# 5l1v3r1/gr-dvbt2ll

Hardware: NVIDIA B200
Metric: t2_baseband_msps (higher is better)
Workload: dtype u8/f32

## Files before the change

gr-dvbt2ll_b200/csrc/t2_capi.cu:

```cuda
#include "../../include/dvbt2ll_cuda.h"

#include <cuda_runtime.h>

#include <algorithm>
#include <cmath>
#include <cstdio>
#include <cstdlib>
#include <cstring>
#include <memory>
#include <mutex>
#include <string>
#include <vector>

#include "t2_kernels.cuh"
#include "t2_plan.h"

namespace {

thread_local std::string g_err;

int fail(int code, const std::string &msg) { g_err = msg; return code; }

#define CK(call)                                                                                  \
  do {                                                                                            \
// ... 549 lines not shown
    t2k::GatherArgs a;
    a.in = (const float2 *)d_in; a.in_stride = plan.stream_items;
    a.out = (float2 *)d_out; a.out_stride = plan.mapped_items;
    a.code = d_code.as<int32_t>(); a.n = plan.mapped_items; a.pool = d_pool.as<float2>();
    a.l1post_base = plan.pool.l1post_base; a.l1post_cells = plan.pool.l1post_cells; a.l1post_variants = plan.pool.l1post_variants;
    a.frames = frames; a.frame_idx0 = t2_frame_num;
    t2k::launch_gather(a, s);
    CK(cudaGetLastError());
    t2_frame_num = (t2_frame_num + frames) % plan.prm.t2frames;
    if (consumed) *consumed = frames * plan.stream_items;
    return frames * plan.mapped_items;
  }
  long long plan_get(const char *name, void *out, long long cap) const
  {
    std::string n(name);
    if (n == "frame.code") return copy_vec(plan.code, out, cap);
    if (n == "frame.pool") return copy_vec(plan.pool.cells, out, cap);
    if (n == "frame.cell_perm") return copy_vec(plan.cell_perm, out, cap);
    if (n == "frame.fec_shift") return copy_vec(plan.fec_shift, out, cap);
    if (n == "frame.ci_dst") return copy_vec(plan.ci_dst, out, cap);
    if (n == "frame.ti_src") return copy_vec(plan.ti_src, out, cap);
    if (n == "frame.dims") return dims_get(plan.dims, out, cap);
    if (n == "frame.info") {
      const int v[12] = { plan.cell_size, plan.stream_items, plan.mapped_items, plan.eta_mod, plan.n_post, plan.n_punc,
                          plan.dummy_cells, plan.pool.l1post_base, plan.pool.l1post_cells, plan.pool.l1post_variants,
                          plan.pool_dummy, plan.pool_zero };
      return copy_out(v, sizeof(v), out, cap);
    }
    return -1;
  }
};

struct OfdmDevice {
  DevBuf d_code, d_pool, d_p1, d_sinc, d_tw, d_tw_split, d_scratch, d_sym_flags;
  int log2_m, split;
  long long pool_stride;
  long long scratch_slot_elems;
  int init(const std::vector<int32_t> &code, const t2::CellPool &pool, const t2::OfdmPlan &op, bool c16 = false)
  {
    {
      const int nv = pool.l1post_variants > 0 ? pool.l1post_variants : 1;
      pool_stride = (long long)pool.cells.size();
      std::vector<t2::cfloat> rep((size_t)nv * pool.cells.size());
      for (int v = 0; v < nv; v++) {
        std::copy(pool.cells.begin(), pool.cells.end(), rep.begin() + (size_t)v * pool.cells.size());
        for (int i = 0; i < pool.l1post_cells; i++)
          rep[(size_t)v * pool.cells.size() + pool.l1post_base + i] = pool.cells[pool.l1post_base + (size_t)v * pool.l1post_cells + i];
      }
      CK(upload(d_pool, rep));
    }
    CK(upload(d_p1, op.p1));
    const int N = op.dims.fft_n;
    split = N > 16384 ? 2 : 1;
    {
      const char *e = std::getenv("DVBT2LL_OFDM_SPLIT16K");
      if (c16 && N == 16384 && e && e[0] == '1') split = 2;
    }
    scratch_slot_elems = 0;
    const int M = N / split;
    log2_m = 0;
    while ((1 << log2_m) < M) log2_m++;
    const int L = op.dims.num_symbols, cps = op.dims.c_ps;
    std::vector<int> pos(M);
    for (int m = 0; m < M; m++) pos[m] = t2k::ofdm_table_index(t2k::ofdm_position_of_bin(m, log2_m), log2_m);
    std::vector<int32_t> code_pos((size_t)L * N, -1);
    std::vector<int32_t> sym_flags(L, 0);
    for (int l = 0; l < L; l++)
      for (int p = 0; p < split; p++)
        for (int m = 0; m < M; m++) {
          const int c = (split * m + p + N / 2) & (N - 1);
          const int k = c - op.left_nulls;
          int32_t v = (k >= 0 && k < cps) ? code[(size_t)l * cps + k] : -1;
          if (c16) {
            if (v >= 0) {
              if (v >= 65536) return fail(DVBT2LL_ERR_INVALID, "chain: staging slot out of range");
              v = 2 * v;
            }
            else if (~v < 8) v = (~v + 1) << 17;
            else { v = (int32_t)(0x80000000u | (uint32_t)(~v)); sym_flags[l] = 1; }
          }
          code_pos[((size_t)l * split + p) * M + pos[m]] = v;
        }
    CK(upload(d_code, code_pos));
    CK(upload(d_sym_flags, sym_flags));
    if (!op.inv_sinc.empty()) {
      std::vector<float> sinc_pos((size_t)N);
      for (int p = 0; p < split; p++)
        for (int m = 0; m < M; m++) sinc_pos[(size_t)p * M + pos[m]] = op.inv_sinc[(split * m + p + N / 2) & (N - 1)];
      CK(upload(d_sinc, sinc_pos));
    }
    CK(upload(d_tw, make_twiddles(M, M)));
    if (split == 2) {
      CK(upload(d_tw_split, make_twiddles(N, M)));
      int dev = 0, sms = 148;
      cudaGetDevice(&dev);
      cudaDeviceGetAttribute(&sms, cudaDevAttrMultiProcessorCount, dev);
      scratch_slot_elems = (long long)(4 * sms + 8) * M;
      CK(d_scratch.ensure((size_t)2 * scratch_slot_elems * sizeof(float2)));
    }
    return 0;
  }
  void fill(t2k::OfdmArgs &a, const t2::OfdmPlan &op, const t2::CellPool &pool) const
  {
    a.code_pos = d_code.as<int32_t>(); a.pool = d_pool.as<float2>(); a.pool_stride = pool_stride;
    a.l1post_base = pool.l1post_base; a.l1post_cells = pool.l1post_cells; a.l1post_variants = pool.l1post_variants;
    a.p1 = d_p1.as<float2>(); a.sinc_pos = op.inv_sinc.empty() ? 0 : d_sinc.as<float>();
    a.tw = d_tw.as<float2>(); a.tw_split = split == 2 ? d_tw_split.as<float2>() : 0;
    a.fft_n = op.dims.fft_n; a.log2_m = log2_m; a.split = split;
    a.c_ps = op.dims.c_ps; a.left_nulls = op.left_nulls; a.gi = op.dims.gi; a.num_symbols = op.dims.num_symbols;
    a.norm = op.normalization;
    a.cells16 = 0; a.run_desc = 0; a.run_ptr = 0; a.run_cnt = 0; a.desc_cap = 0; a.stage_bytes = 0; a.stage_cap = 0; a.lut = 0; a.lut_n = 0; a.lut_single = 0;
    a.sym_flags = d_sym_flags.as<int32_t>();
    a.out_fmt = 0; a.sink_gain = 1.0f; a.scratch = d_scratch.as<float2>();
    a.cells_len = 0; a.out_len = 0; a.pool_len = pool_stride;
  }
};

struct OfdmHandle : dvbt2ll_handle {
  t2::OfdmPlan plan;
  OfdmDevice dev;
  OfdmHandle() : dvbt2ll_handle(OFDM) {}
  int output_multiple() const { return plan.samples_per_frame; }
  int in_item() const { return 8; }
  int out_item() const { return 8; }
  int forecast(int noutput) const { return plan.dims.active_items * (noutput / plan.samples_per_frame); }
  int dev_init() { return dev.init(plan.code, plan.pool, plan); }
  int work_device(const void *d_in, int ninput, void *d_out, int noutput, int *consumed, cudaStream_t s)
  {
    const int frames = noutput / plan.samples_per_frame;
    if (consumed) *consumed = 0;
    if (frames < 1) return 0;
    if ((long long)ninput < (long long)frames * plan.dims.active_items)
      return fail(DVBT2LL_ERR_SHORT, "pilotgenp1insert_cc: not enough input items");
    t2k::OfdmArgs a;
    dev.fill(a, plan, plan.pool);
    a.cells = (const float2 *)d_in; a.cells_stride = plan.dims.active_items;
    a.out = d_out; a.out_stride = plan.samples_per_frame;
    a.cells_len = (long long)frames * plan.dims.active_items; a.out_len = (long long)frames * plan.samples_per_frame;
    a.frames = frames; a.frame_idx0 = 0; a.frames_per_channel = frames;
    t2k::launch_ofdm(a, s);
    CK(cudaGetLastError());
    if (consumed) *consumed = frames * plan.dims.active_items;
    return frames * plan.samples_per_frame;
  }
  long long plan_get(const char *name, void *out, long long cap) const
  {
// ... 86 lines not shown
    int r;
    if ((r = bb.dev_init())) return r;
    if ((r = ldpc.dev_init())) return r;
    if ((r = map.dev_init())) return r;
    if ((r = odev.init(tables.code, tables.pool, oplan, true))) return r;
    CK(upload(d_ci_inv, fplan.cell_perm_inv));
    {
      const int nc = (int)fplan.cell_perm_inv.size();
      ci4_stride = (nc + 8 + 3) & ~3;
      std::vector<uint16_t> c4((size_t)4 * ci4_stride, 0);
      for (int k = 0; k < 4; k++)
        for (int j = 0; j + k < nc; j++) {
          const int c = fplan.cell_perm_inv[j + k];
          c4[(size_t)k * ci4_stride + j] = (uint16_t)(c + 2 * (c >> 6));
        }
      CK(upload(d_ci_inv4, c4));
    }
    CK(upload(d_fec_shift, fplan.fec_shift));
    CK(upload(d_run_desc, tables.run_desc));
    CK(upload(d_run_ptr, tables.run_ptr));
    CK(upload(d_run_cnt, tables.run_cnt));
    CK(upload(d_stage_bytes, tables.stage_bytes));
    stage_cap = (tables.max_slots + 7) & ~7;
    if ((size_t)(1 << odev.log2_m) * 8 * 17 / 16 + (size_t)stage_cap * 2 + 2048 + 96 + (size_t)(tables.max_runs + 2) * 8 > 227 * 1024)
      return fail(DVBT2LL_ERR_INVALID, "chain: the cells of one OFDM symbol do not fit the shared-memory staging area");
    const size_t nfec = (size_t)max_frames * F();
    CK(d_bch.ensure(nfec * align16(bb.plan.fec.nbch / 8) + 64));
    CK(d_cells.ensure((size_t)max_frames * cells16_stride() * sizeof(uint16_t) + 64));
    CK(cudaMemset(d_cells.p, 0, (size_t)max_frames * cells16_stride() * sizeof(uint16_t) + 64));
    for (int s = 0; s < TIMING_SLOTS; s++) for (int i = 0; i < 5; i++) CK(cudaEventCreate(&ev[s][i]));
    return 0;
  }
  int run(const void *d_ts, long long ts_pitch, int n_channels, int n_frames, long long first_frame, void *d_out, cudaStream_t s,
          int buf_frame = 0, int scratch_slot = 0, int hist_valid = -1)
  {
    const int frames = n_channels * n_frames;
    if (frames < 1) return 0;
    if (buf_frame + frames > max_frames) return fail(DVBT2LL_ERR_INVALID, "chain: batch larger than max_frames given at create");
    const int nfec = frames * F();
    const int bp = align16(bb.plan.fec.nbch / 8), fp = align16(bb.plan.fec.nldpc / 8);
    cudaEvent_t *tev = ev[n_timed % TIMING_SLOTS];
    if (timing) cudaEventRecord(tev[0], s);
    uint8_t *bch_buf = d_bch.as<uint8_t>() + (size_t)buf_frame * F() * bp;
    if (!fuse_fec || taps) CK(d_fec.ensure((size_t)max_frames * F() * fp + 64));
    uint8_t *fec_buf = d_fec.as<uint8_t>() ? d_fec.as<uint8_t>() + (size_t)buf_frame * F() * fp : 0;
    uint16_t *cell_buf = d_cells.as<uint16_t>() + (size_t)buf_frame * cells16_stride();
    for (int pl = 0; pl < P(); pl++) {
      const int fpl = Fp(pl);
      const long long j0 = first_frame * fpl;
      const int fb0 = bb.plan.inband ? (int)(j0 % fpl) : 0;
      const int count0 = (int)(stream_pos(first_frame, pl) % 188);
      t2k::BbArgs ba;
      bb.fill_args(ba, (const uint8_t *)d_ts + (long long)pl * ts_pitch, ts_pitch * P(), n_channels, n_frames * fpl, count0, fb0,
                   hist_valid >= 0 ? hist_valid : (first_frame > 0 ? 1 : 0), bch_buf, bp);
      ba.fecblocks = fpl;
      ba.ts_len = ts_bytes(first_frame, n_frames, pl);
      ba.out_len = (long long)frames * F() * bp;
      if (P() > 1) { ba.out_group = fpl; ba.out_group_stride = F(); ba.out_group_off = fplan.plp_first_block[pl]; }
      t2k::launch_bb_bch(ba, s);
    }
    if (timing) cudaEventRecord(tev[1], s);
    t2k::LdpcArgs la;
    ldpc.fill_args(la, bch_buf, bp, fec_buf, fp, nfec);
    t2k::MapArgs ma;
    map.fill_args(ma, fec_buf, fp, 0, nfec);
    ma.out16 = cell_buf; ma.out16_frame_stride = cells16_stride();
    ma.ci_inv = d_ci_inv.as<uint16_t>(); ma.fec_shift = d_fec_shift.as<int32_t>(); ma.fecblocks = F();
    ma.ci_inv4 = d_ci_inv4.as<uint16_t>(); ma.ci_inv4_stride = ci4_stride;
    ma.out_len = (long long)frames * cells16_stride();
    if (fuse_fec) {
      if (timing) cudaEventRecord(tev[2], s);
      t2k::launch_fec(la, ma, taps ? fec_buf : 0, fp, s);
    }
    else {
      t2k::launch_ldpc(la, s);
      if (timing) cudaEventRecord(tev[2], s);
      t2k::launch_map(ma, s);
    }
    if (timing) cudaEventRecord(tev[3], s);
    t2k::OfdmArgs oa;
    odev.fill(oa, oplan, tables.pool);
    oa.cells = 0; oa.cells_stride = cells16_stride();
    oa.cells16 = cell_buf; oa.run_desc = d_run_desc.as<int2>(); oa.run_ptr = d_run_ptr.as<int32_t>();
    oa.run_cnt = d_run_cnt.as<int32_t>(); oa.desc_cap = (tables.max_runs + 2) & ~1;
    oa.stage_bytes = d_stage_bytes.as<int32_t>(); oa.stage_cap = stage_cap; oa.lut_single = map.plan.im_from_re;
    oa.lut = map.d_lut.as<float2>(); oa.lut_n = 1 << map.plan.mod;
    oa.out = d_out; oa.out_stride = oplan.samples_per_frame;
    oa.cells_len = (long long)frames * cells16_stride(); oa.out_len = (long long)frames * oplan.samples_per_frame;
    oa.out_fmt = sink_fmt; oa.sink_gain = sink_gain; oa.norm = oplan.normalization * sink_gain;
    if (oa.scratch && scratch_slot) oa.scratch += odev.scratch_slot_elems;
    oa.frames = frames; oa.frames_per_channel = n_frames;
    oa.frame_idx0 = (int)(first_frame % (tables.pool.l1post_variants > 0 ? tables.pool.l1post_variants : 1));
    t2k::launch_ofdm(oa, s);
    if (timing) { cudaEventRecord(tev[4], s); n_timed++; }
    CK(cudaGetLastError());
    if (buf_frame == 0) last_frames = frames;
    return frames;
  }
  int work_device(const void *d_in, int ninput, void *d_out, int noutput, int *consumed, cudaStream_t s)
  {
    const int frames = noutput / oplan.samples_per_frame;
    if (consumed) *consumed = 0;
    if (frames < 1) return 0;
    const long long need = ts_bytes(next_frame, frames);
    if ((long long)ninput < need) return fail(DVBT2LL_ERR_SHORT, "chain: not enough input items");
    int r = run(d_in, 0, 1, frames, next_frame, d_out, s);
    if (r < 0) return r;
    next_frame += frames;
    if (consumed) *consumed = (int)need;
    return frames * oplan.samples_per_frame;
  }
  long long plan_get(const char *name, void *out, long long cap) const
  {
    std::string n(name);
    if (n == "chain.code") return copy_vec(tables.code, out, cap);
    if (n == "chain.pool") return copy_vec(tables.pool.cells, out, cap);
    if (n == "chain.run_desc") return copy_vec(tables.run_desc, out, cap);
    if (n == "chain.run_ptr") return copy_vec(tables.run_ptr, out, cap);
    if (n == "chain.run_cnt") return copy_vec(tables.run_cnt, out, cap);
    if (n == "chain.stage_bytes") return copy_vec(tables.stage_bytes, out, cap);
    if (n == "ofdm.sym_data_start") return copy_vec(oplan.sym_data_start, out, cap);
    if (n == "frame.framed") return copy_vec(fplan.framed, out, cap);
    if (n == "frame.pool") return copy_vec(fplan.pool.cells, out, cap);
// ... 156 lines not shown
  LinkRec::Slot *mine = 0;
  if (h->link_out) {
    LinkRec &L = *h->link_out;
    mine = &L.slot[L.next];
    if ((r = write_back(L, *mine)) < 0) return r;
    for (int k = 0; k < LinkRec::NSLOT; k++) {
      LinkRec::Slot &S = L.slot[k];
      if (&S != mine && S.valid && (const uint8_t *)out < S.host + S.bytes && (const uint8_t *)out + out_bytes > S.host) {
        if ((r = write_back(L, S)) < 0) return r;
        S.valid = false;
      }
    }
    if (mine->taken_valid) CK(cudaStreamWaitEvent(h->stream, mine->taken_ev, 0));
    mine->valid = false;
    for (int k = 0; k < LinkRec::NSLOT; k++)
      if (!L.slot[k].valid) CK(L.slot[k].buf.ensure(out_bytes + 256));
    lk_out.unlock();
  }
  if (lk_in.owns_lock() && !resident) lk_in.unlock();
  DevBuf &d_out = mine ? mine->buf : h->stage_out;
  if (!resident) CK(d_in.ensure(prefix + in_bytes + 256));
  CK(d_out.ensure(out_bytes + 256));
  uint8_t *din = resident ? const_cast<uint8_t *>(resident) : d_in.as<uint8_t>() + prefix;
  cudaStream_t s = h->stream;
  if (!resident) h->pin(in, in_bytes);
  h->pin(out, out_bytes);
  if (b) {
    CK(cudaMemcpyAsync(din - 187, b->history, 187, cudaMemcpyHostToDevice, s));
    b->hist_on_device = 1;
  }
  if (!resident) CK(h->copy_host(din, in, in_bytes, cudaMemcpyHostToDevice, s));
  int used = 0;
  if (ch) {
    r = ch->run(din, 0, 1, frames, ch->next_frame, d_out.p, s, 0, 0, 1);
    if (r >= 0) { r = nout; used = (int)need; ch->next_frame += frames; }
  }
  else r = h->work_device(din, (int)need, d_out.p, nout, &used, s);
  if (r < 0) return r;
  if (resident) {
    if (!taken->taken_ev) CK(cudaEventCreateWithFlags(&taken->taken_ev, cudaEventDisableTiming));
    CK(cudaEventRecord(taken->taken_ev, s));
    taken->taken_valid = true;
    lk_in.unlock();
  }
  const bool lazy_out = h->link_out && h->link_out->lazy;
  if (!lazy_out) CK(h->copy_host(out, d_out.p, out_bytes, cudaMemcpyDeviceToHost, s));
  CK(cudaStreamSynchronize(s));
  if (b) {
    h->warnings = *b->h_err;
    b->note_consumed((const uint8_t *)in, used);
  }
  if (mine) {
    lk_out.lock();
    LinkRec &L = *h->link_out;
    mine->host = (const uint8_t *)out; mine->bytes = out_bytes; mine->valid = true;
    mine->pending = lazy_out; mine->taken_to = 0;
    L.next = (L.next + 1) % LinkRec::NSLOT;
  }
  if (consumed) *consumed = used;
  return r;
}

long long dvbt2ll_ts_sync(const unsigned char *ts, size_t n)
{
  if (!ts) return -1;
  for (size_t off = 0; off < 188 && off < n; off++) {
    int ok = 0;
// ... 236 lines not shown
{
  ChainHandle *c = as_chain(h);
  if (!c) return fail(DVBT2LL_ERR_INVALID, "not a chain handle");
  int r = c->enter();
  if (r) return r;
  if (n_channels < 0 || n_frames < 0) return fail(DVBT2LL_ERR_INVALID, "chain: negative batch size");
  if (n_channels == 0 || n_frames == 0) return 0;
  const int P = c->P();
  const long long per_ch = c->ts_bytes_max(first_frame, n_frames);
  const long long hist = (first_frame > 0 && c->bb.plan.mode == t2::INPUTMODE_NORMAL) ? 187 : 0;
  if (n_channels * P == 1 && ts_pitch < per_ch + hist) ts_pitch = per_ch + hist;
  if (ts_pitch < per_ch + hist)
    return fail(DVBT2LL_ERR_INVALID, "chain: ts_pitch smaller than the TS bytes (+ 187 history bytes) of one channel");
  const long long dpitch = (per_ch + hist + 255) & ~255LL;
  const size_t ssz = c->sink_fmt ? 4 : 8;
  const size_t out_bytes = (size_t)n_channels * n_frames * c->oplan.samples_per_frame * ssz;
  CK(c->d_ts_stage.ensure((size_t)n_channels * P * dpitch + 512));
  CK(c->d_out_stage.ensure(out_bytes));
  uint8_t *base = c->d_ts_stage.as<uint8_t>() + 256;
  uint8_t *dout = c->d_out_stage.as<uint8_t>();
  const size_t ch_out = (size_t)n_frames * c->oplan.samples_per_frame;
  if (!c->stream2) CK(cudaStreamCreateWithFlags(&c->stream2, cudaStreamNonBlocking));
  int groups = n_channels >= 8 ? 8 : n_channels;
  while (groups > 1 && 2 * ((n_channels + groups - 1) / groups) * n_frames > c->max_frames) groups--;
  const int per = (n_channels + groups - 1) / groups;
  if (2 * per * n_frames > c->max_frames) groups = 1;
  int gi = 0;
  for (int c0 = 0; c0 < n_channels; c0 += (groups == 1 ? n_channels : per), gi++) {
    const int nc = groups == 1 ? n_channels : (c0 + per <= n_channels ? per : n_channels - c0);
    cudaStream_t s = (gi & 1) ? c->stream2 : c->stream;
    CK(cudaMemcpy2DAsync(base + (size_t)c0 * P * dpitch - hist, (size_t)dpitch, (const uint8_t *)ts + (size_t)c0 * P * ts_pitch - hist,
                         (size_t)ts_pitch, (size_t)(per_ch + hist), (size_t)nc * P, cudaMemcpyHostToDevice, s));
    r = c->run(base + (size_t)c0 * P * dpitch, dpitch, nc, n_frames, first_frame, dout + (size_t)c0 * ch_out * ssz, s,
               groups == 1 ? 0 : (gi & 1) * per * n_frames, gi & 1);
    if (r < 0) return r;
    CK(cudaMemcpyAsync((uint8_t *)out + (size_t)c0 * ch_out * ssz, dout + (size_t)c0 * ch_out * ssz, (size_t)nc * ch_out * ssz,
                       cudaMemcpyDeviceToHost, s));
  }
  CK(cudaStreamSynchronize(c->stream));
  CK(cudaStreamSynchronize(c->stream2));
  return n_channels * n_frames;
}

long long dvbt2ll_chain_tap(dvbt2ll_handle *h, const char *stage, void *out, long long cap)
{
  ChainHandle *c = as_chain(h);
  if (!c || !stage) return fail(DVBT2LL_ERR_INVALID, "not a chain handle");
  if (!c->dev_ready || c->last_frames < 1) return fail(DVBT2LL_ERR_INVALID, "chain: nothing has run yet");
  const size_t nfec = (size_t)c->last_frames * c->F();
  const void *src; size_t bytes;
  std::string n(stage);
  if (n == "bch") { src = c->d_bch.p; bytes = nfec * align16(c->bb.plan.fec.nbch / 8); }
  else if (n == "fec") {
    if (c->fuse_fec && !c->taps) return fail(DVBT2LL_ERR_INVALID, "chain: the LDPC codewords stay on chip; call dvbt2ll_chain_enable_taps before the run");
    src = c->d_fec.p; bytes = nfec * align16(c->bb.plan.fec.nldpc / 8);
  }
  else if (n == "cells") { src = c->d_cells.p; bytes = (size_t)c->last_frames * c->cells16_stride() * sizeof(uint16_t); }
  else return fail(DVBT2LL_ERR_INVALID, "chain: unknown tap");
  CK(cudaStreamSynchronize(c->stream));
  CK(cudaDeviceSynchronize());
  if (out && cap > 0) CK(cudaMemcpy(out, src, (size_t)cap < bytes ? (size_t)cap : bytes, cudaMemcpyDeviceToHost));
  return (long long)bytes;
}

int dvbt2ll_chain_set_sink(dvbt2ll_handle *h, int format, float gain)
{
  ChainHandle *c = as_chain(h);
// ... 42 lines not shown
```

gr-dvbt2ll_b200/csrc/t2_kernels.cu:

```cuda
#include "t2_kernels.cuh"

#include <atomic>

#ifdef DVBT2LL_DEBUG_BOUNDS
#include <cstdio>
#define BND(ok)                                                                                                   \
  do {                                                                                                            \
    if (!(ok)) {                                                                                                  \
      printf("DVBT2LL bounds violation: %s (t2_kernels.cu:%d, block %d thread %d)\n", #ok, __LINE__, (int)blockIdx.x, (int)threadIdx.x); \
      __trap();                                                                                                   \
    }                                                                                                             \
  } while (0)
#else
#define BND(ok) do { } while (0)
#endif

namespace t2k {

static std::atomic<long long> g_launches(0);
long long kernel_launch_count() { return g_launches.load(); }
static inline void count_launch() { g_launches.fetch_add(1); }
void count_extra_launch() { count_launch(); }

constexpr int MAX_DEVICES = 64;
// ... 1633 lines not shown
          const unsigned sc = *reinterpret_cast<const uint16_t *>(stage + off);
          const unsigned esh = 2 + lut_rep_shift, emask = 255u << esh, lane_off = (threadIdx.x & ((1u << lut_rep_shift) - 1u)) << 2;
          float2 val = make_float2(*reinterpret_cast<const float *>(reinterpret_cast<const uint8_t *>(lut_re) + (((sc << esh) & emask) | lane_off)),
                                   *reinterpret_cast<const float *>(reinterpret_cast<const uint8_t *>(lut_im) + ((((sc >> 8) << esh) & emask) | lane_off)));
          if (cc >= 0x20000) val = *reinterpret_cast<const float2 *>(spool_m8 + ((unsigned)cc >> 14));
#endif
          if (POOL && cc < 0) val = __ldg(pool + (cc & 0x7FFFFFFF));
          v[b][r] = val;
        }
        else {
          const float2 *base = cc >= 0 ? cells : pool;
          v[b][r] = __ldg(base + (cc >= 0 ? cc : ~cc));
        }
      }
    if (g0 + G::STEP < G::GROUPS) fill_load_codes<LOG2M, T>(code, g0 + G::STEP, c);
#pragma unroll
    for (int b = 0; b < GPB; b++) {
      const int g = g0 + b * T;
      if (SINC) {
#pragma unroll
        for (int r = 0; r < R0; r++) {
          const float sf = __ldg(sinc + (R0 == 16 ? (((r >> 2) * G::GROUPS + g) * 4 + (r & 3)) : g * R0 + r));
          v[b][r] = __fmul2_rn(v[b][r], make_float2(sf, sf));
        }
      }
      if (R0 > 1) dft_reg<R0>(v[b]);
      float2 *xb = x + padx(g * R0);
#pragma unroll
      for (int k = 0; k < R0; k++) xb[k] = v[b][bitrev_c(k, R0)];
    }
  }
}

template <int LOG2M, int T, bool C16, int FMT, int SPLIT>
__global__ void __launch_bounds__(T, (LOG2M == 14 ? 1 : 1024 / T)) k_ofdm(const OfdmArgs a)
{
  extern __shared__ __align__(16) uint8_t smem_raw[];
  float2 *x = reinterpret_cast<float2 *>(smem_raw);
  constexpr int M = 1 << LOG2M;
  uint8_t *stage = reinterpret_cast<uint8_t *>(x + padx(M));
  float *lut_re = reinterpret_cast<float *>(stage + 2 * a.stage_cap);
  const int lut_rep_shift = a.lut_rep_shift, lut_rep = 1 << lut_rep_shift;
  const int lut_e = a.lut_n < 16 ? 16 : a.lut_n;
  float *lut_im = a.lut_single ? lut_re : lut_re + lut_e * lut_rep;
  float2 *spool = reinterpret_cast<float2 *>(lut_re + (a.lut_single ? lut_e : 2 * lut_e) * lut_rep);
  uint64_t *mbar = reinterpret_cast<uint64_t *>(spool + 8);
  const uint32_t mbar_s = (uint32_t)__cvta_generic_to_shared(mbar), dbar_s = mbar_s + 8;
  const int2 *descbuf = reinterpret_cast<const int2 *>(mbar + 2);
  const uint32_t desc_s = mbar_s + 16;
  if (C16) {
    if (threadIdx.x < a.lut_n) x[threadIdx.x] = __ldg(a.lut + threadIdx.x);
    if (threadIdx.x < 8) spool[threadIdx.x] = __ldg(a.pool + threadIdx.x);
    if (threadIdx.x < 4) reinterpret_cast<uint32_t *>(stage)[threadIdx.x] = 0u;
    if (threadIdx.x == 0) {
      asm volatile("mbarrier.init.shared::cta.b64 [%0], 1;\n" ::"r"(mbar_s) : "memory");
      asm volatile("mbarrier.init.shared::cta.b64 [%0], 1;\n" ::"r"(dbar_s) : "memory");
      asm volatile("fence.mbarrier_init.release.cluster;\n" ::: "memory");
    }
    __syncthreads();
    for (int i = threadIdx.x; i < a.lut_n * lut_rep; i += T) {
      const float2 v = x[i >> lut_rep_shift];
      lut_re[i] = v.x;
      if (!a.lut_single) lut_im[i] = v.y;
    }
    __syncthreads();
  }
  constexpr int R0 = FillGeom<LOG2M, T>::R0;
  constexpr int NLAST = M / 16;
  const int N = a.fft_n;
  const int units = a.frames * a.num_symbols;
  const int cp_from = N - a.gi;
  const uint32_t stage_s = (uint32_t)__cvta_generic_to_shared(stage);
  FillSmem fs;
  fs.stage_s = stage_s;
  fs.esh = 2u + (uint32_t)lut_rep_shift;
  fs.lut_lane_s = (uint32_t)__cvta_generic_to_shared(lut_re) + ((threadIdx.x & (uint32_t)(lut_rep - 1)) << 2);
  fs.im_ofs = a.lut_single ? 0u : 4u * (uint32_t)(lut_e * lut_rep);
  fs.spool_m8_s = (uint32_t)__cvta_generic_to_shared(spool) - 8u;
  constexpr bool REGTW = LOG2M == 14;
  static_assert(!REGTW || T == 512, "the 16K schedule is written for 512 threads");
  float2 tw_p1 = make_float2(1.f, 0.f), tw_p2 = tw_p1, tw_last = tw_p1, tw_rec = tw_p1;
  if (REGTW) {
    tw_p1 = __ldg(a.tw + (threadIdx.x & 15) * (M / 256));
    tw_p2 = __ldg(a.tw + (threadIdx.x & 255) * (M / 4096));
    tw_last = __ldg(a.tw + threadIdx.x);
    if (SPLIT == 2) tw_rec = __fmul2_rn(__ldg(a.tw_split + threadIdx.x), make_float2(a.norm, a.norm));
  }
  constexpr bool PRETW = !REGTW && (M / 16 <= T);
  constexpr int NP1 = R0, NP2 = R0 * 16 < NLAST ? R0 * 16 : 1;
  (void)NP1; (void)NP2;
  if (PRETW) {
#ifndef OFDM_NO_PRETW
    tw_p1 = __ldg(a.tw + (threadIdx.x & (NP1 - 1)) * (M / (NP1 * 16)));
    tw_p2 = __ldg(a.tw + (threadIdx.x & (NP2 - 1)) * (M / (NP2 * 16)));
    tw_last = (int)threadIdx.x < NLAST ? __ldg(a.tw + threadIdx.x) : make_float2(1.f, 0.f);
#endif
  }

  uint32_t mphase = 0, dphase = 0;
// ... 27 lines not shown
    for (int i = threadIdx.x; i < rr.y; i += T) {
      const int2 d = descbuf[i];
      BND(i < a.desc_cap);
      BND(((unsigned)d.y >> 16) + ((unsigned)d.y & 0xFFFFu) <= (unsigned)a.stage_cap / 8u && d.x >= 0);
      BND(a.cells_len == 0 || (long long)uf * a.cells_stride * 2 + 16ll * (d.x + (d.y & 0xFFFF)) <= a.cells_len * 2 + 64);
      asm volatile("cp.async.bulk.shared::cluster.global.mbarrier::complete_tx::bytes [%0], [%1], %2, [%3];\n"
                   ::"r"(stage_s + 16u * ((uint32_t)d.y >> 16)), "l"(src + 16ll * d.x), "r"(16u * ((uint32_t)d.y & 0xFFFFu)), "r"(mbar_s) : "memory");
    }
  };
  auto stage_wait = [&]() {
    uint32_t done;
    do {
      asm volatile("{\n.reg .pred p;\nmbarrier.try_wait.parity.shared::cta.b64 p, [%1], %2;\nselp.u32 %0, 1, 0, p;\n}\n"
                   : "=r"(done) : "r"(mbar_s), "r"(mphase) : "memory");
    } while (!done);
    mphase ^= 1u;
  };

  int2 cp0 = make_int2(0, 0), cp1 = cp0;
  if (C16 && (int)blockIdx.x < units) {
    cp0 = run_range(blockIdx.x);
    if (threadIdx.x == 0) desc_issue(cp0);
  }
  for (int unit = blockIdx.x; unit < units; unit += gridDim.x) {
    const int f = unit / a.num_symbols, l = unit - f * a.num_symbols;
    if (C16 && unit + (int)gridDim.x < units) cp1 = run_range(unit + gridDim.x);
    const int variant = (a.frame_idx0 + (f % a.frames_per_channel)) % a.l1post_variants;
    const float2 *cells = a.cells + (long long)f * a.cells_stride;
    const float2 *pool = a.pool + (long long)variant * a.pool_stride;
    typedef typename SinkT<FMT>::type sample_t;
    sample_t *out = reinterpret_cast<sample_t *>(a.out) + (long long)f * a.out_stride;
    sample_t *sym = out + 2048 + (long long)l * (N + a.gi);
    BND(a.out_len == 0 || (long long)f * a.out_stride + 2048 + (long long)(l + 1) * (N + a.gi) <= a.out_len);
    float2 *park = FMT == 0 ? reinterpret_cast<float2 *>(sym) + a.gi : a.scratch + (long long)blockIdx.x * M;

    if (l == 0)
      for (int i = threadIdx.x; i < 2048; i += T) {
        float2 p = __ldg(a.p1 + i);
        p.x *= a.sink_gain; p.y *= a.sink_gain;
        store_sample(out, i, p);
      }

    bool pool_sym = false;
    if (C16) pool_sym = __ldg(a.sym_flags + l) != 0;
    int c[FillGeom<LOG2M, T>::GPB][FillGeom<LOG2M, T>::R0];
    fill_load_codes<LOG2M, T>(a.code_pos + (long long)l * SPLIT * M, threadIdx.x, c);
    if (C16) {
      if (unit == (int)blockIdx.x) stage_issue(unit, cp0);
      if (cp0.y > 0) stage_wait();
    }

    for (int phase = 0; phase < SPLIT; phase++) {
      const int32_t *code = a.code_pos + ((long long)l * SPLIT + phase) * M;
      const float *sinc = a.sinc_pos ? a.sinc_pos + (long long)phase * M : nullptr;
      const uint8_t *spool_m8 = reinterpret_cast<const uint8_t *>(spool) - 8;
      if (phase) fill_load_codes<LOG2M, T>(code, threadIdx.x, c);
      __syncthreads();
      if (C16 && phase == 0 && threadIdx.x == 0 && unit + (int)gridDim.x < units) desc_issue(cp1);
      if (sinc) {
        if (pool_sym) ofdm_fill<LOG2M, T, C16, true, true>(x, code, sinc, c, stage, lut_re, lut_im, lut_rep_shift, spool_m8, cells, pool, fs, a.stage_cap);
        else ofdm_fill<LOG2M, T, C16, false, true>(x, code, sinc, c, stage, lut_re, lut_im, lut_rep_shift, spool_m8, cells, pool, fs, a.stage_cap);
      }
      else {
        if (pool_sym) ofdm_fill<LOG2M, T, C16, true, false>(x, code, sinc, c, stage, lut_re, lut_im, lut_rep_shift, spool_m8, cells, pool, fs, a.stage_cap);
        else ofdm_fill<LOG2M, T, C16, false, false>(x, code, sinc, c, stage, lut_re, lut_im, lut_rep_shift, spool_m8, cells, pool, fs, a.stage_cap);
      }
      __syncthreads();
      if (C16 && phase == SPLIT - 1) {
        if (unit + (int)gridDim.x < units) stage_issue(unit + gridDim.x, cp1);
        cp0 = cp1;
      }
      if constexpr (REGTW) {
#ifdef OFDM_PASS_TREE
        fft_pass16<M, 16, T, REGTW>(x, a.tw, tw_p1); __syncthreads();
        fft_pass16<M, 256, T, REGTW>(x, a.tw, tw_p2); __syncthreads();
#else
        fft_pass16x2<M, 16, T>(x, tw_p1); __syncthreads();
        fft_pass16x2<M, 256, T>(x, tw_p2); __syncthreads();
#endif
      }
      else {
#ifndef OFDM_NO_PRETW
        if (R0 * 16 < NLAST * 16 && R0 < NLAST) { fft_pass16<M, NP1, T, PRETW>(x, a.tw, tw_p1); __syncthreads(); }
        if (R0 * 16 < NLAST) { fft_pass16<M, NP2, T, PRETW>(x, a.tw, tw_p2); __syncthreads(); }
#else
        if (R0 * 16 < NLAST * 16 && R0 < NLAST) { fft_pass16<M, R0, T>(x, a.tw); __syncthreads(); }
        if (R0 * 16 < NLAST) { fft_pass16<M, (R0 * 16 < NLAST ? R0 * 16 : 1), T>(x, a.tw); __syncthreads(); }
#endif
      }
      if constexpr (REGTW) {
        constexpr int NL = M / 4, NBT = NL / T;
        constexpr int XS = NL + NL / 16;
        sample_t *o = sym + a.gi + threadIdx.x;
        const bool odd_phase = SPLIT == 2 && phase == 1;
        const float2 *pk = park + threadIdx.x;
#ifndef PARK_AHEAD
#define PARK_AHEAD 1
#endif
        float2 e[PARK_AHEAD + 1][4];
        if (odd_phase) {
#pragma unroll
          for (int jj = 0; jj < PARK_AHEAD; jj++)
#pragma unroll
            for (int k = 0; k < 4; k++) e[jj][k] = pk[jj * T + k * NL];
        }
#pragma unroll
        for (int j = 0; j < NBT; j++) {
          const int i = threadIdx.x + j * T;
          const float2 *xb = x + padx(i);
          float2 v[4];
#pragma unroll
          for (int q = 0; q < 4; q++) v[q] = xb[q * XS];
          if (odd_phase && j + PARK_AHEAD < NBT) {
#pragma unroll
            for (int k = 0; k < 4; k++) e[(j + PARK_AHEAD) % (PARK_AHEAD + 1)][k] = pk[(j + PARK_AHEAD) * T + k * NL];
          }
          const float2 w1 = j ? cmul(tw_last, w32(j)) : tw_last;
          const float2 w2 = cmul(w1, w1), w3 = cmul(w2, w1);
          v[1] = cmul(v[1], w1); v[2] = cmul(v[2], w2); v[3] = cmul(v[3], w3);
          dft_reg<4>(v);
          if (SPLIT == 1) {
            sample_t *ocp = sym + ((long long)threadIdx.x - cp_from);
#pragma unroll
            for (int k = 0; k < 4; k++) {
              const float2 r = __fmul2_rn(v[bitrev_c(k, 4)], make_float2(a.norm, a.norm));
              store_sample(o, j * T + k * NL, r);
              if (i + k * NL >= cp_from) store_sample(ocp, j * T + k * NL, r);
            }
          }
          else if (phase == 0) {
            float2 *pw = park + threadIdx.x;
#pragma unroll
            for (int k = 0; k < 4; k++) pw[j * T + k * NL] = __fmul2_rn(v[bitrev_c(k, 4)], make_float2(a.norm, a.norm));
          }
          else {
            sample_t *ocp = sym + ((long long)threadIdx.x + M - cp_from);
            const float2 wi = j ? cmul(tw_rec, w64(j)) : tw_rec;
#pragma unroll
            for (int k = 0; k < 4; k++) {
              const float2 r = cmul(tw16(v[bitrev_c(k, 4)], 2 * k), wi);
              store_sample(o, j * T + k * NL, cadd(e[j % (PARK_AHEAD + 1)][k], r));
              const float2 hi = csub(e[j % (PARK_AHEAD + 1)][k], r);
              store_sample(o, j * T + k * NL + M, hi);
              if (i + k * NL + M >= cp_from) store_sample(ocp, j * T + k * NL, hi);
            }
          }
        }
      }
      else
#pragma unroll 1
      for (int i = threadIdx.x; i < NLAST; i += T) {
        const float2 *xb = x + padx(i);
#ifndef OFDM_NO_PRETW
        const float2 w1 = PRETW ? tw_last : __ldg(a.tw + i);
#else
        const float2 w1 = __ldg(a.tw + i);
#endif
        float2 v[16];
#pragma unroll
        for (int qd = 0; qd < 16; qd++) v[qd] = xb[padx(qd * NLAST)];
        apply_twiddles<16>(v, w1);
        dft_reg<16>(v);
        sample_t *o = sym + a.gi + i;
        if (SPLIT == 1) {
          sample_t *ocp = sym + ((long long)i - cp_from);
#pragma unroll
          for (int k = 0; k < 16; k++) {
            float2 r = v[bitrev_c(k, 16)];
            r = __fmul2_rn(r, make_float2(a.norm, a.norm));
            store_sample(o, k * NLAST, r);
            if (i + k * NLAST >= cp_from) store_sample(ocp, k * NLAST, r);
          }
        }
        else if (phase == 0) {
          float2 *pk = park + i;
#pragma unroll
          for (int k = 0; k < 16; k++) {
            float2 r = v[bitrev_c(k, 16)];
            r = __fmul2_rn(r, make_float2(a.norm, a.norm));
            pk[k * NLAST] = r;
          }
        }
        else {
          const float2 *pk = park + i;
          sample_t *ocp = sym + ((long long)i + M - cp_from);
          const float2 wi = __fmul2_rn(__ldg(a.tw_split + i), make_float2(a.norm, a.norm));
#pragma unroll
          for (int h = 0; h < 2; h++) {
            float2 e[8];
#pragma unroll
            for (int k = 0; k < 8; k++) e[k] = pk[(8 * h + k) * NLAST];
#pragma unroll
            for (int k = 0; k < 8; k++) {
              const int kk = 8 * h + k;
              const float2 r = cmul(cmul(v[bitrev_c(kk, 16)], w32(kk)), wi);
              store_sample(o, kk * NLAST, cadd(e[k], r));
              const float2 hi = csub(e[k], r);
              store_sample(o, kk * NLAST + M, hi);
              if (i + kk * NLAST + M >= cp_from) store_sample(ocp, kk * NLAST, hi);
            }
          }
        }
      }
    }
  }
}

static inline size_t lut_table_bytes(const OfdmArgs &a) { return (size_t)(a.lut_n < 16 ? 16 : a.lut_n) * 4 * (a.lut_single ? 1 : 2); }

template <int LOG2M, int T, bool C16, int FMT, int SPLIT>
static void launch_ofdm_t(const OfdmArgs &a, cudaStream_t s)
{
  constexpr int M = 1 << LOG2M;
  const size_t smem = (size_t)padx(M) * sizeof(float2) +
                      (C16 ? (size_t)a.stage_cap * 2 + ((size_t)lut_table_bytes(a) << a.lut_rep_shift) + 64 + 16 + (size_t)a.desc_cap * 8 : 0);
  const int units = a.frames * a.num_symbols;
  static bool attr[MAX_DEVICES];
  allow_smem(k_ofdm<LOG2M, T, C16, FMT, SPLIT>, 227 * 1024, attr);
  int per_sm = 1;
  cudaOccupancyMaxActiveBlocksPerMultiprocessor(&per_sm, k_ofdm<LOG2M, T, C16, FMT, SPLIT>, T, smem);
  if (per_sm < 1) per_sm = 1;
  int blocks = sm_count() * per_sm;
  if (blocks > units) blocks = units;
  k_ofdm<LOG2M, T, C16, FMT, SPLIT><<<blocks, T, smem, s>>>(a);
  count_launch();
}

template <bool C16, int FMT>
static void launch_ofdm_c(const OfdmArgs &a, cudaStream_t s)
{
  switch (a.log2_m) {
    case 10: launch_ofdm_t<10, 256, C16, FMT, 1>(a, s); break;
    case 11: launch_ofdm_t<11, 256, C16, FMT, 1>(a, s); break;
    case 12: launch_ofdm_t<12, 256, C16, FMT, 1>(a, s); break;
    case 13:
      if (a.split == 2) launch_ofdm_t<13, 512, C16, FMT, 2>(a, s);
      else launch_ofdm_t<13, 512, C16, FMT, 1>(a, s);
      break;
    case 14:
      if (a.split == 2) launch_ofdm_t<14, 512, C16, FMT, 2>(a, s);
      else launch_ofdm_t<14, 512, C16, FMT, 1>(a, s);
      break;
    default: break;
  }
}

void launch_ofdm(const OfdmArgs &a0, cudaStream_t s)
{
  if (a0.frames * a0.num_symbols < 1) return;
  OfdmArgs a = a0;
  a.lut_rep_shift = 0;
  if (a.cells16) {
    const size_t base = (size_t)padx(1 << a.log2_m) * sizeof(float2) + (size_t)a.stage_cap * 2 + 64 + 16 + (size_t)a.desc_cap * 8, sm_bytes = 227 * 1024;
    const size_t one = lut_table_bytes(a);
    size_t ctas = sm_bytes / (base + one + 1024);
    if (ctas < 1) ctas = 1;
    if (ctas > 2) ctas = 2;
    for (int sh = 5; sh > 0; sh--)
      if (base + (one << sh) + 1024 <= sm_bytes / ctas) { a.lut_rep_shift = sh; break; }
  }
  if (a.cells16) {
    if (a.out_fmt) launch_ofdm_c<true, 1>(a, s);
    else launch_ofdm_c<true, 0>(a, s);
  }
  else launch_ofdm_c<false, 0>(a, s);
}

}
```

gr-dvbt2ll_b200/csrc/t2_kernels.cuh:

```cuda
#ifndef T2_KERNELS_CUH
#define T2_KERNELS_CUH

#include <cuda_runtime.h>
#include <stdint.h>

namespace t2k {

struct BbArgs {
  const uint8_t *ts;
  long long ts_pitch;
  int hist_valid;
  int n_channels, frames;
  int count0;
  int fec_block0;
  int kbch, nbch, bch_r, payload_bytes, mode, inband, fecblocks;
  int chunk_bytes, lead_zero_bytes;
  const uint8_t *scramble;
  const uint8_t *crc8_tab;
  uint32_t crc8_mask[8];
  uint32_t crc8_pos_mask[47][8];
  const uint32_t *bch_tab;
  const uint32_t *bch_cols;
  const uint8_t *inband_bytes;
  uint8_t *out;
// ... 48 lines not shown
void launch_pack_bits(const uint8_t *in, int nbits, uint8_t *out, int out_pitch, int frames, cudaStream_t s);
void launch_unpack_bits(const uint8_t *in, int in_pitch, int nbits, uint8_t *out, int frames, cudaStream_t s);
void launch_unpack_ldpc(const uint8_t *in, int in_pitch, int nbch, int nldpc, int q, uint8_t *out, int frames,
                        cudaStream_t s);
void launch_pack_ldpc(const uint8_t *in, int nbch, int nldpc, int q, uint8_t *out, int out_pitch, int frames,
                      cudaStream_t s);

struct GatherArgs {
  const float2 *in;  long long in_stride;
  float2 *out;       long long out_stride;
  const int32_t *code; int n;
  const float2 *pool;
  int l1post_base, l1post_cells, l1post_variants;
  int frames; int frame_idx0;
};
void launch_gather(const GatherArgs &a, cudaStream_t s);

struct OfdmArgs {
  const float2 *cells; long long cells_stride;
  const uint16_t *cells16;
  const int2 *run_desc;
  const int32_t *run_ptr;
  const int32_t *run_cnt;
  int desc_cap;
  const int32_t *stage_bytes;
  const int32_t *sym_flags;
  int stage_cap;
  const float2 *lut; int lut_n;
  int lut_single;
  int lut_rep_shift;
  void *out;           long long out_stride;
  int out_fmt;
  float sink_gain;
  float2 *scratch;
  const int32_t *code_pos;
  const float2 *pool;
  long long pool_stride;
  int l1post_base, l1post_cells, l1post_variants;
  const float2 *p1;
  const float *sinc_pos;
  const float2 *tw;
  const float2 *tw_split;
  int fft_n, log2_m, split;
  int c_ps, left_nulls, gi, num_symbols;
  float norm;
  int frames; int frame_idx0;
  int frames_per_channel;
  long long cells_len, out_len, pool_len;
};
void launch_ofdm(const OfdmArgs &a, cudaStream_t s);
int ofdm_position_of_bin(int m, int log2_m);
int ofdm_table_index(int p, int log2_m);

long long kernel_launch_count();

}
#endif
```

Measured before the change: 125,300.

## Park split-FFT first-half results in tensor memory instead of global scratch

For 32K symbols transformed as two 16K halves, the first-phase outputs were previously parked in global memory (the output buffer or a per-block scratch slot) and re-read in the second phase. The kernel now allocates 256 TMEM columns per CTA and stores and loads these intermediates with tcgen05.st/ld, which removes the scratch buffer, its slot bookkeeping, and the 16K split option. This cuts global memory round-trips, but adds TMEM allocation and fence overhead per block and may limit occupancy.

```diff
diff --git a/gr-dvbt2ll_b200/csrc/t2_capi.cu b/gr-dvbt2ll_b200/csrc/t2_capi.cu
--- a/gr-dvbt2ll_b200/csrc/t2_capi.cu
+++ b/gr-dvbt2ll_b200/csrc/t2_capi.cu
@@ -605,10 +605,9 @@
 };
 
 struct OfdmDevice {
-  DevBuf d_code, d_pool, d_p1, d_sinc, d_tw, d_tw_split, d_scratch, d_sym_flags;
+  DevBuf d_code, d_pool, d_p1, d_sinc, d_tw, d_tw_split, d_sym_flags;
   int log2_m, split;
   long long pool_stride;
-  long long scratch_slot_elems;
   int init(const std::vector<int32_t> &code, const t2::CellPool &pool, const t2::OfdmPlan &op, bool c16 = false)
   {
     {
@@ -625,11 +624,6 @@
     CK(upload(d_p1, op.p1));
     const int N = op.dims.fft_n;
     split = N > 16384 ? 2 : 1;
-    {
-      const char *e = std::getenv("DVBT2LL_OFDM_SPLIT16K");
-      if (c16 && N == 16384 && e && e[0] == '1') split = 2;
-    }
-    scratch_slot_elems = 0;
     const int M = N / split;
     log2_m = 0;
     while ((1 << log2_m) < M) log2_m++;
@@ -663,14 +657,7 @@
       CK(upload(d_sinc, sinc_pos));
     }
     CK(upload(d_tw, make_twiddles(M, M)));
-    if (split == 2) {
-      CK(upload(d_tw_split, make_twiddles(N, M)));
-      int dev = 0, sms = 148;
-      cudaGetDevice(&dev);
-      cudaDeviceGetAttribute(&sms, cudaDevAttrMultiProcessorCount, dev);
-      scratch_slot_elems = (long long)(4 * sms + 8) * M;
-      CK(d_scratch.ensure((size_t)2 * scratch_slot_elems * sizeof(float2)));
-    }
+    if (split == 2) CK(upload(d_tw_split, make_twiddles(N, M)));
     return 0;
   }
   void fill(t2k::OfdmArgs &a, const t2::OfdmPlan &op, const t2::CellPool &pool) const
@@ -684,7 +671,7 @@
     a.norm = op.normalization;
     a.cells16 = 0; a.run_desc = 0; a.run_ptr = 0; a.run_cnt = 0; a.desc_cap = 0; a.stage_bytes = 0; a.stage_cap = 0; a.lut = 0; a.lut_n = 0; a.lut_single = 0;
     a.sym_flags = d_sym_flags.as<int32_t>();
-    a.out_fmt = 0; a.sink_gain = 1.0f; a.scratch = d_scratch.as<float2>();
+    a.out_fmt = 0; a.sink_gain = 1.0f;
     a.cells_len = 0; a.out_len = 0; a.pool_len = pool_stride;
   }
 };
@@ -837,7 +824,7 @@
     return 0;
   }
   int run(const void *d_ts, long long ts_pitch, int n_channels, int n_frames, long long first_frame, void *d_out, cudaStream_t s,
-          int buf_frame = 0, int scratch_slot = 0, int hist_valid = -1)
+          int buf_frame = 0, int hist_valid = -1)
   {
     const int frames = n_channels * n_frames;
     if (frames < 1) return 0;
@@ -893,7 +880,6 @@
     oa.out = d_out; oa.out_stride = oplan.samples_per_frame;
     oa.cells_len = (long long)frames * cells16_stride(); oa.out_len = (long long)frames * oplan.samples_per_frame;
     oa.out_fmt = sink_fmt; oa.sink_gain = sink_gain; oa.norm = oplan.normalization * sink_gain;
-    if (oa.scratch && scratch_slot) oa.scratch += odev.scratch_slot_elems;
     oa.frames = frames; oa.frames_per_channel = n_frames;
     oa.frame_idx0 = (int)(first_frame % (tables.pool.l1post_variants > 0 ? tables.pool.l1post_variants : 1));
     t2k::launch_ofdm(oa, s);
@@ -1116,7 +1102,7 @@
   if (!resident) CK(h->copy_host(din, in, in_bytes, cudaMemcpyHostToDevice, s));
   int used = 0;
   if (ch) {
-    r = ch->run(din, 0, 1, frames, ch->next_frame, d_out.p, s, 0, 0, 1);
+    r = ch->run(din, 0, 1, frames, ch->next_frame, d_out.p, s, 0, 1);
     if (r >= 0) { r = nout; used = (int)need; ch->next_frame += frames; }
   }
   else r = h->work_device(din, (int)need, d_out.p, nout, &used, s);
@@ -1419,7 +1405,7 @@
     CK(cudaMemcpy2DAsync(base + (size_t)c0 * P * dpitch - hist, (size_t)dpitch, (const uint8_t *)ts + (size_t)c0 * P * ts_pitch - hist,
                          (size_t)ts_pitch, (size_t)(per_ch + hist), (size_t)nc * P, cudaMemcpyHostToDevice, s));
     r = c->run(base + (size_t)c0 * P * dpitch, dpitch, nc, n_frames, first_frame, dout + (size_t)c0 * ch_out * ssz, s,
-               groups == 1 ? 0 : (gi & 1) * per * n_frames, gi & 1);
+               groups == 1 ? 0 : (gi & 1) * per * n_frames);
     if (r < 0) return r;
     CK(cudaMemcpyAsync((uint8_t *)out + (size_t)c0 * ch_out * ssz, dout + (size_t)c0 * ch_out * ssz, (size_t)nc * ch_out * ssz,
                        cudaMemcpyDeviceToHost, s));
diff --git a/gr-dvbt2ll_b200/csrc/t2_kernels.cu b/gr-dvbt2ll_b200/csrc/t2_kernels.cu
--- a/gr-dvbt2ll_b200/csrc/t2_kernels.cu
+++ b/gr-dvbt2ll_b200/csrc/t2_kernels.cu
@@ -1689,6 +1689,39 @@
   }
 }
 
+constexpr int OFDM_PARK_COLS = 256;
+
+template <int NCOLS>
+__device__ __forceinline__ void tmem_alloc(uint32_t dst_s)
+{
+  asm volatile("tcgen05.alloc.cta_group::1.sync.aligned.shared::cta.b32 [%0], %1;\n" ::"r"(dst_s), "n"(NCOLS) : "memory");
+}
+__device__ __forceinline__ void tmem_relinquish() { asm volatile("tcgen05.relinquish_alloc_permit.cta_group::1.sync.aligned;\n" ::: "memory"); }
+template <int NCOLS>
+__device__ __forceinline__ void tmem_dealloc(uint32_t taddr)
+{
+  asm volatile("tcgen05.dealloc.cta_group::1.sync.aligned.b32 %0, %1;\n" ::"r"(taddr), "n"(NCOLS) : "memory");
+}
+__device__ __forceinline__ void tmem_fence_before_sync() { asm volatile("tcgen05.fence::before_thread_sync;\n" ::: "memory"); }
+__device__ __forceinline__ void tmem_fence_after_sync() { asm volatile("tcgen05.fence::after_thread_sync;\n" ::: "memory"); }
+__device__ __forceinline__ void tmem_st4(uint32_t taddr, const float2 (&v)[4])
+{
+  asm volatile("tcgen05.st.sync.aligned.32x32b.x8.b32 [%0], {%1, %2, %3, %4, %5, %6, %7, %8};\n"
+               ::"r"(taddr), "f"(v[0].x), "f"(v[0].y), "f"(v[1].x), "f"(v[1].y), "f"(v[2].x), "f"(v[2].y), "f"(v[3].x), "f"(v[3].y));
+}
+__device__ __forceinline__ void tmem_wait_st() { asm volatile("tcgen05.wait::st.sync.aligned;\n" ::: "memory"); }
+__device__ __forceinline__ void tmem_ld4(uint32_t taddr, float2 (&v)[4])
+{
+  asm volatile("tcgen05.ld.sync.aligned.32x32b.x8.b32 {%0, %1, %2, %3, %4, %5, %6, %7}, [%8];\n"
+               : "=f"(v[0].x), "=f"(v[0].y), "=f"(v[1].x), "=f"(v[1].y), "=f"(v[2].x), "=f"(v[2].y), "=f"(v[3].x), "=f"(v[3].y)
+               : "r"(taddr));
+}
+__device__ __forceinline__ void tmem_wait_ld4(float2 (&v)[4])
+{
+  asm volatile("tcgen05.wait::ld.sync.aligned;\n"
+               : "+f"(v[0].x), "+f"(v[0].y), "+f"(v[1].x), "+f"(v[1].y), "+f"(v[2].x), "+f"(v[2].y), "+f"(v[3].x), "+f"(v[3].y));
+}
+
 template <int LOG2M, int T, bool C16, int FMT, int SPLIT>
 __global__ void __launch_bounds__(T, (LOG2M == 14 ? 1 : 1024 / T)) k_ofdm(const OfdmArgs a)
 {
@@ -1722,6 +1755,20 @@
     }
     __syncthreads();
   }
+  static_assert(SPLIT == 1 || LOG2M == 14, "only 32K symbols are transformed as two halves");
+  uint32_t park_col = 0;
+  if constexpr (SPLIT == 2) {
+    uint32_t *tm_slot = reinterpret_cast<uint32_t *>(x);
+    if (threadIdx.x < 32) {
+      tmem_alloc<OFDM_PARK_COLS>((uint32_t)__cvta_generic_to_shared(tm_slot));
+      tmem_relinquish();
+    }
+    tmem_fence_before_sync();
+    __syncthreads();
+    tmem_fence_after_sync();
+    const uint32_t warp = threadIdx.x >> 5;
+    park_col = *tm_slot + ((32u * (warp & 3u)) << 16) + 64u * (warp >> 2);
+  }
   constexpr int R0 = FillGeom<LOG2M, T>::R0;
   constexpr int NLAST = M / 16;
   const int N = a.fft_n;
@@ -1815,7 +1862,6 @@
     sample_t *out = reinterpret_cast<sample_t *>(a.out) + (long long)f * a.out_stride;
     sample_t *sym = out + 2048 + (long long)l * (N + a.gi);
     BND(a.out_len == 0 || (long long)f * a.out_stride + 2048 + (long long)(l + 1) * (N + a.gi) <= a.out_len);
-    float2 *park = FMT == 0 ? reinterpret_cast<float2 *>(sym) + a.gi : a.scratch + (long long)blockIdx.x * M;
 
     if (l == 0)
       for (int i = threadIdx.x; i < 2048; i += T) {
@@ -1876,28 +1922,16 @@
         constexpr int XS = NL + NL / 16;
         sample_t *o = sym + a.gi + threadIdx.x;
         const bool odd_phase = SPLIT == 2 && phase == 1;
-        const float2 *pk = park + threadIdx.x;
-#ifndef PARK_AHEAD
-#define PARK_AHEAD 1
-#endif
-        float2 e[PARK_AHEAD + 1][4];
-        if (odd_phase) {
-#pragma unroll
-          for (int jj = 0; jj < PARK_AHEAD; jj++)
-#pragma unroll
-            for (int k = 0; k < 4; k++) e[jj][k] = pk[jj * T + k * NL];
-        }
+        if (odd_phase) tmem_wait_st();
 #pragma unroll
         for (int j = 0; j < NBT; j++) {
           const int i = threadIdx.x + j * T;
           const float2 *xb = x + padx(i);
+          float2 e[4];
+          if (odd_phase) tmem_ld4(park_col + 8u * j, e);
           float2 v[4];
 #pragma unroll
           for (int q = 0; q < 4; q++) v[q] = xb[q * XS];
-          if (odd_phase && j + PARK_AHEAD < NBT) {
-#pragma unroll
-            for (int k = 0; k < 4; k++) e[(j + PARK_AHEAD) % (PARK_AHEAD + 1)][k] = pk[(j + PARK_AHEAD) * T + k * NL];
-          }
           const float2 w1 = j ? cmul(tw_last, w32(j)) : tw_last;
           const float2 w2 = cmul(w1, w1), w3 = cmul(w2, w1);
           v[1] = cmul(v[1], w1); v[2] = cmul(v[2], w2); v[3] = cmul(v[3], w3);
@@ -1912,18 +1946,22 @@
             }
           }
           else if (phase == 0) {
-            float2 *pw = park + threadIdx.x;
-#pragma unroll
-            for (int k = 0; k < 4; k++) pw[j * T + k * NL] = __fmul2_rn(v[bitrev_c(k, 4)], make_float2(a.norm, a.norm));
+            float2 r[4];
+#pragma unroll
+            for (int k = 0; k < 4; k++) r[k] = __fmul2_rn(v[bitrev_c(k, 4)], make_float2(a.norm, a.norm));
+            tmem_st4(park_col + 8u * j, r);
           }
           else {
             sample_t *ocp = sym + ((long long)threadIdx.x + M - cp_from);
             const float2 wi = j ? cmul(tw_rec, w64(j)) : tw_rec;
+            float2 r[4];
+#pragma unroll
+            for (int k = 0; k < 4; k++) r[k] = cmul(tw16(v[bitrev_c(k, 4)], 2 * k), wi);
+            tmem_wait_ld4(e);
 #pragma unroll
             for (int k = 0; k < 4; k++) {
-              const float2 r = cmul(tw16(v[bitrev_c(k, 4)], 2 * k), wi);
-              store_sample(o, j * T + k * NL, cadd(e[j % (PARK_AHEAD + 1)][k], r));
-              const float2 hi = csub(e[j % (PARK_AHEAD + 1)][k], r);
+              store_sample(o, j * T + k * NL, cadd(e[k], r[k]));
+              const float2 hi = csub(e[k], r[k]);
               store_sample(o, j * T + k * NL + M, hi);
               if (i + k * NL + M >= cp_from) store_sample(ocp, j * T + k * NL, hi);
             }
@@ -1945,46 +1983,23 @@
         apply_twiddles<16>(v, w1);
         dft_reg<16>(v);
         sample_t *o = sym + a.gi + i;
-        if (SPLIT == 1) {
-          sample_t *ocp = sym + ((long long)i - cp_from);
-#pragma unroll
-          for (int k = 0; k < 16; k++) {
-            float2 r = v[bitrev_c(k, 16)];
-            r = __fmul2_rn(r, make_float2(a.norm, a.norm));
-            store_sample(o, k * NLAST, r);
-            if (i + k * NLAST >= cp_from) store_sample(ocp, k * NLAST, r);
-          }
+        sample_t *ocp = sym + ((long long)i - cp_from);
+#pragma unroll
+        for (int k = 0; k < 16; k++) {
+          float2 r = v[bitrev_c(k, 16)];
+          r = __fmul2_rn(r, make_float2(a.norm, a.norm));
+          store_sample(o, k * NLAST, r);
+          if (i + k * NLAST >= cp_from) store_sample(ocp, k * NLAST, r);
         }
-        else if (phase == 0) {
-          float2 *pk = park + i;
-#pragma unroll
-          for (int k = 0; k < 16; k++) {
-            float2 r = v[bitrev_c(k, 16)];
-            r = __fmul2_rn(r, make_float2(a.norm, a.norm));
-            pk[k * NLAST] = r;
-          }
-        }
-        else {
-          const float2 *pk = park + i;
-          sample_t *ocp = sym + ((long long)i + M - cp_from);
-          const float2 wi = __fmul2_rn(__ldg(a.tw_split + i), make_float2(a.norm, a.norm));
-#pragma unroll
-          for (int h = 0; h < 2; h++) {
-            float2 e[8];
-#pragma unroll
-            for (int k = 0; k < 8; k++) e[k] = pk[(8 * h + k) * NLAST];
-#pragma unroll
-            for (int k = 0; k < 8; k++) {
-              const int kk = 8 * h + k;
-              const float2 r = cmul(cmul(v[bitrev_c(kk, 16)], w32(kk)), wi);
-              store_sample(o, kk * NLAST, cadd(e[k], r));
-              const float2 hi = csub(e[k], r);
-              store_sample(o, kk * NLAST + M, hi);
-              if (i + kk * NLAST + M >= cp_from) store_sample(ocp, kk * NLAST, hi);
-            }
-          }
-        }
-      }
+      }
+    }
+  }
+  if constexpr (SPLIT == 2) {
+    tmem_fence_before_sync();
+    __syncthreads();
+    if (threadIdx.x < 32) {
+      tmem_fence_after_sync();
+      tmem_dealloc<OFDM_PARK_COLS>(park_col);
     }
   }
 }
@@ -2016,10 +2031,7 @@
     case 10: launch_ofdm_t<10, 256, C16, FMT, 1>(a, s); break;
     case 11: launch_ofdm_t<11, 256, C16, FMT, 1>(a, s); break;
     case 12: launch_ofdm_t<12, 256, C16, FMT, 1>(a, s); break;
-    case 13:
-      if (a.split == 2) launch_ofdm_t<13, 512, C16, FMT, 2>(a, s);
-      else launch_ofdm_t<13, 512, C16, FMT, 1>(a, s);
-      break;
+    case 13: launch_ofdm_t<13, 512, C16, FMT, 1>(a, s); break;
     case 14:
       if (a.split == 2) launch_ofdm_t<14, 512, C16, FMT, 2>(a, s);
       else launch_ofdm_t<14, 512, C16, FMT, 1>(a, s);
diff --git a/gr-dvbt2ll_b200/csrc/t2_kernels.cuh b/gr-dvbt2ll_b200/csrc/t2_kernels.cuh
--- a/gr-dvbt2ll_b200/csrc/t2_kernels.cuh
+++ b/gr-dvbt2ll_b200/csrc/t2_kernels.cuh
@@ -104,7 +104,6 @@
   void *out;           long long out_stride;
   int out_fmt;
   float sink_gain;
-  float2 *scratch;
   const int32_t *code_pos;
   const float2 *pool;
   long long pool_stride;
```

Result: faster. 129,800, median of 6 (+3.6%).
